# Zanue/EndoDAV

Measured on AMD Instinct MI355X. Metric: depth frames/sec (518x518, T=8 clip), higher is better.
Workload: dtype f32

## Files before the change

endodav_amd/_lib.py:

```python
from __future__ import annotations

import ctypes as C
import os
from typing import Optional

_HERE = os.path.dirname(os.path.abspath(__file__))
LIB_PATH = os.environ.get("EDV_LIB_PATH") or os.path.join(_HERE, "lib", "libendodav_hip.so")
ABI_VERSION = 15

LORA_TYPES = {"none": 0, "lora": 1, "dvlora": 2, "ssb": 3, "dash": 4}
ACT_NONE, ACT_GELU, ACT_RELU, ACT_SIGMOID, ACT_SIGMOID_NEG = 0, 1, 2, 3, 4


class EdvConfig(C.Structure):

    _fields_ = [
        ("abi_version", C.c_int32),
        ("embed_dim", C.c_int32),
        ("depth", C.c_int32),
        ("num_heads", C.c_int32),
        ("taps", C.c_int32 * 4),
        ("features", C.c_int32),
        ("out_channels", C.c_int32 * 4),
        ("image_h", C.c_int32),
# ... 29 lines not shown
    "edv_forward": (C.c_int, [C.c_void_p, _fp, _i32, _i32, _i32, _i32, C.POINTER(C.c_void_p), C.c_void_p]),
    "edv_output_shape": (C.c_int, [C.c_void_p, _i32, C.POINTER(_i32), C.POINTER(_i32)]),
    "edv_stage_copy": (C.c_int, [C.c_void_p, C.c_char_p, _fp, C.POINTER(C.c_size_t), C.c_void_p]),
    "edv_set_capture": (C.c_int, [C.c_void_p, C.c_int]),
    "edv_profile_enable": (C.c_int, [C.c_void_p, C.c_uint32]),
    "edv_set_encoder_streams": (C.c_int, [C.c_void_p, _i32]),
    "edv_set_products": (C.c_int, [C.c_void_p, _i32, C.c_void_p]),
    "edv_get_products": (C.c_int, [C.c_void_p]),
    "edv_profile_set_mask": (C.c_int, [C.c_void_p, C.c_uint32]),
    "edv_profile_work": (C.c_int, [C.c_void_p, _i32, C.POINTER(_f64), C.POINTER(_f64)]),
    "edv_profile_read": (C.c_int, [C.c_void_p, _i32, C.POINTER(_i32), C.POINTER(_f64)]),
    "edv_device_bytes": (C.c_size_t, [C.c_void_p]),
    "edv_last_launch_count": (C.c_int, [C.c_void_p]),
    "edv_layernorm": (C.c_int, [_fp, _fp, _fp, _fp, _i64, _i32, _f32, _fp, _i32, _i32, C.c_void_p]),
    "edv_gemm_workspace": (C.c_size_t, []),
    "edv_gemm_x6_planes_bytes": (C.c_size_t, [_i32, _i32]),
    "edv_gemm_x6_split": (C.c_int, [_fp, C.c_void_p, _i32, _i32, C.c_void_p]),
    "edv_gemm_x6": (C.c_int, [_fp, C.c_void_p, _fp, _i64, _i32, _i32, _fp, _i32, _fp, _fp, _fp, C.c_size_t, C.c_void_p]),
    "edv_gemm": (C.c_int, [_fp, _fp, _fp, _i64, _i32, _i32, _fp, _i32, _fp, _fp, _fp, C.c_size_t, C.c_void_p]),
    "edv_pack_geglu": (C.c_int, [_fp, _fp, _fp, _fp, _i32, _i32, C.c_void_p]),
    "edv_gemm_geglu": (C.c_int, [_fp, _fp, _fp, _fp, _i64, _i32, _i32, C.c_void_p]),
    "edv_conv3x3": (C.c_int, [_fp, _fp, _fp, _fp, _i32, _i32, _i32, _i32, _i32, _i32, _i32, _i32, _fp, _fp, C.c_void_p]),
    "edv_conv3x3_ws": (C.c_int, [_fp, _fp, _fp, _fp, _i32, _i32, _i32, _i32, _i32, _i32, _i32, _i32, _fp, _fp, _fp, C.c_size_t, C.c_void_p]),
    "edv_pack_conv3x3": (C.c_int, [_fp, _fp, _i32, _i32, C.c_void_p]),
    "edv_conv_transpose": (C.c_int, [_fp, _fp, _fp, _fp, _fp, _fp, _i32, _i32, _i32, _i32, _i32, C.c_void_p]),
    "edv_attn_spatial_workspace": (C.c_size_t, [_i32, _i32, _i32]),
    "edv_attn_spatial": (C.c_int, [_fp, _fp, _i32, _i32, _i32, _fp, C.c_size_t, _fp, C.c_void_p]),
    "edv_set_train": (C.c_int, [C.c_void_p, _i32]),
    "edv_set_grad_scope": (C.c_int, [C.c_void_p, _i32, _i32, _i32, _i32]),
    "edv_set_bias_grads": (C.c_int, [C.c_void_p, _i32, _i32]),
    "edv_generation": (C.c_int, [C.c_void_p, C.POINTER(C.c_uint64)]),
    "edv_backward": (C.c_int, [C.c_void_p, C.c_uint64, _fp, C.POINTER(C.c_void_p), C.c_void_p]),
    "edv_grad_bind_flat": (C.c_int, [C.c_void_p, _i32, C.POINTER(C.c_char_p), C.POINTER(_i64), _fp, _i64, C.POINTER(_i64)]),
    "edv_grad": (C.c_int, [C.c_void_p, C.c_char_p, C.POINTER(C.c_void_p), C.POINTER(_i64)]),
    "edv_grad_copy": (C.c_int, [C.c_void_p, C.c_char_p, _fp, _i64, C.c_void_p]),
    "edv_attn_spatial_x6_workspace": (C.c_size_t, [_i32, _i32, _i32]),
    "edv_attn_spatial_x6": (C.c_int, [_fp, _fp, _i32, _i32, _i32, _fp, C.c_size_t, C.c_void_p]),
    "edv_attn_spatial_bwd_workspace": (C.c_size_t, [_i32, _i32, _i32]),
    "edv_attn_spatial_bwd": (C.c_int, [_fp, _fp, _fp, _fp, _fp, _fp, _i32, _i32, _i32, _fp, C.c_size_t, C.c_void_p]),
    "edv_layernorm_bwd": (C.c_int, [_fp, _fp, _fp, _fp, _i64, _i32, C.c_float, _i32, C.c_void_p]),
    "edv_ew_bwd": (C.c_int, [_fp, _fp, _fp, _fp, _i64, _i32, C.c_void_p]),
    "edv_geglu_bwd": (C.c_int, [_fp, _fp, _fp, _i64, _i32, C.c_void_p]),
    "edv_transpose_scale": (C.c_int, [_fp, _fp, _fp, _i32, _i32, C.c_void_p]),
    "edv_lora_grads_workspace": (C.c_size_t, [_i64, _i32, _i32, _i32]),
    "edv_lora_grads": (C.c_int, [_fp, _fp, _i64, _i32, _i32, _i32, _fp, _fp, _fp, _fp, C.c_float, _fp, _fp, C.c_size_t, _fp, _fp, _fp, _fp, C.c_void_p]),
    "edv_bilinear_bwd": (C.c_int, [_fp, _fp, _i32, _i32, _i32, _i32, _i32, _i32, _i32, C.c_void_p]),
# ... 128 lines not shown
```

endodav_amd/csrc/api.hip:

```cpp
#include "../../include/endodav_hip.h"
#include <algorithm>
#include <vector>

#include "ops.hpp"

using namespace edv;

extern "C" {

int edv_layernorm(const float *x_dev, const float *w_dev, const float *b_dev, float *y_dev, int64_t rows, int32_t dim, float eps,
                  const float *pe_dev, int32_t rows_per_frame, int32_t T, void *stream) {
    return layernorm(x_dev, identity_map(), w_dev, b_dev, y_dev, identity_map(), rows, dim, eps, pe_dev, rows_per_frame, T, (hipStream_t)stream);
}

size_t edv_gemm_workspace(void) { return gemm_workspace() * sizeof(float); }
int edv_gemm(const float *A_dev, const float *W_dev, float *C_dev, int64_t M, int32_t N, int32_t K, const float *bias_dev, int32_t act,
             const float *gamma_dev, const float *R_dev, float *workspace_dev, size_t workspace_bytes, void *stream) {
    GemmDesc g;
    g.A = A_dev; g.lda = K; g.W = W_dev; g.ldw = K; g.C = C_dev; g.ldc = N; g.M = M; g.N = N; g.K = K;
    g.bias = bias_dev; g.act = act; g.gamma = gamma_dev; g.R1 = R_dev; g.ldr1 = N;
    g.ws = workspace_dev; g.ws_floats = workspace_bytes / sizeof(float);
    EDV_CHECK(act >= ACT_NONE && act <= ACT_RELU, "act must be 0, 1 or 2");
    return gemm(g, (hipStream_t)stream);
}
// ... 33 lines not shown
                        int32_t Cout, int32_t stride, int32_t pre_relu, int32_t post_relu, const float *R1_dev, const float *R2_dev, float *ws,
                        size_t ws_bytes, void *stream) {
    EDV_CHECK(F > 0 && H > 0 && W > 0 && Cin > 0 && Cout > 0, "empty problem");
    EDV_CHECK(stride == 1 || stride == 2, "stride must be 1 or 2");
    GemmDesc g;
    const int OH = (H - 1) / stride + 1, OW = (W - 1) / stride + 1;
    g.A = x_dev; g.W = wpacked_dev; g.ldw = 9 * Cin; g.C = y_dev; g.ldc = Cout; g.M = (long long)F * OH * OW; g.N = Cout; g.K = 9 * Cin;
    g.bias = bias_dev; g.act = post_relu ? ACT_RELU : ACT_NONE; g.R1 = R1_dev; g.ldr1 = Cout; g.R2 = R2_dev; g.ldr2 = Cout;
    g.loader = LOAD_CONV3; g.cH = H; g.cW = W; g.cC = Cin; g.cOH = OH; g.cOW = OW; g.cS = stride; g.pre_relu = pre_relu ? 1 : 0;
    g.ws = ws; g.ws_floats = ws_bytes / sizeof(float);
    return gemm(g, (hipStream_t)stream);
}

int edv_conv3x3(const float *x_dev, const float *wpacked_dev, const float *bias_dev, float *y_dev, int32_t F, int32_t H, int32_t W, int32_t Cin,
                int32_t Cout, int32_t stride, int32_t pre_relu, int32_t post_relu, const float *R1_dev, const float *R2_dev, void *stream) {
    return conv3x3_impl(x_dev, wpacked_dev, bias_dev, y_dev, F, H, W, Cin, Cout, stride, pre_relu, post_relu, R1_dev, R2_dev, nullptr, 0, stream);
}

int edv_conv3x3_ws(const float *x_dev, const float *wpacked_dev, const float *bias_dev, float *y_dev, int32_t F, int32_t H, int32_t W, int32_t Cin,
                   int32_t Cout, int32_t stride, int32_t pre_relu, int32_t post_relu, const float *R1_dev, const float *R2_dev, float *workspace_dev,
                   size_t workspace_bytes, void *stream) {
    return conv3x3_impl(x_dev, wpacked_dev, bias_dev, y_dev, F, H, W, Cin, Cout, stride, pre_relu, post_relu, R1_dev, R2_dev, workspace_dev,
                        workspace_bytes, stream);
}

int edv_pack_conv3x3(const float *w_dev, float *wpacked_dev, int32_t Cout, int32_t Cin, void *stream) {
    return pack_conv3x3(w_dev, wpacked_dev, Cout, Cin, (hipStream_t)stream);
}

int edv_conv_transpose(const float *x_dev, const float *w_dev, const float *b_dev, float *wpack_dev, float *bpack_dev, float *y_dev, int32_t F, int32_t h,
              int32_t w, int32_t C, int32_t s, void *stream) {
    EDV_CHECK(F > 0 && h > 0 && w > 0 && C > 0 && s > 0, "empty problem");
    EDV_TRY(pack_convT(w_dev, wpack_dev, b_dev, bpack_dev, C, C, s, (hipStream_t)stream));
    GemmDesc g;
    g.A = x_dev; g.lda = C; g.W = wpack_dev; g.ldw = C; g.C = y_dev; g.ldc = C; g.M = (long long)F * h * w; g.N = s * s * C; g.K = C;
    g.bias = bpack_dev; g.store = STORE_SHUFFLE; g.ps_s = s; g.ps_C = C; g.ps_h = h; g.ps_w = w;
    return gemm(g, (hipStream_t)stream);
}

size_t edv_attn_spatial_workspace(int32_t F, int32_t N, int32_t heads) { return attn_spatial_workspace(F, N, heads) * sizeof(float); }
int edv_attn_spatial(const float *qkv_dev, float *out_dev, int32_t F, int32_t N, int32_t heads, float *workspace_dev, size_t workspace_bytes,
                     float *lse_dev, void *stream) {
    return attn_spatial(qkv_dev, out_dev, F, N, heads, workspace_dev, workspace_bytes / sizeof(float), (hipStream_t)stream, lse_dev);
}
size_t edv_attn_spatial_x6_workspace(int32_t F, int32_t N, int32_t heads) { return attn_spatial_workspace(F, N, heads, true) * sizeof(float); }
int edv_attn_spatial_x6(const float *qkv_dev, float *out_dev, int32_t F, int32_t N, int32_t heads, float *workspace_dev, size_t workspace_bytes, void *stream) {
// ... 336 lines not shown
```

endodav_amd/csrc/conv_dma.hip:

```cpp
#include <cstdlib>
#include <type_traits>

#include "gemm_common.hpp"

namespace edv {
namespace {

constexpr int CBK = 32;
__device__ __attribute__((aligned(256))) float g_zero_page[64];

template <int WGM, int EP, bool SPLIT, bool BUF>
__global__ __launch_bounds__(256, 4) void conv3_dma_kernel(const GemmDesc g, const GemmSplit sp) {
    constexpr int WGN = 4 / WGM;
    constexpr int BM = 32 * WGM, BN = 32 * WGN;
    constexpr int IA = BM / 32, IB = BN / 32;
    constexpr int STAGE = (BM + BN) * CBK;
    __shared__ __attribute__((aligned(16))) float smem[2 * STAGE];
    const int tid = threadIdx.x, lane = tid & 63, wave = tid >> 6, l31 = lane & 31, lh = lane >> 5;
    const int wave_s = __builtin_amdgcn_readfirstlane(wave);
    const bool prelu = g.pre_relu != 0;
    const int wm = wave / WGN, wn = wave % WGN;
    const int tiles_n = (g.N + BN - 1) / BN;
    const int bid = xcd_remap(blockIdx.x, gridDim.x);
    const unsigned a_bytes = BUF ? (unsigned)((g.M > 0 ? ((g.M - 1) / (g.cOH * g.cOW) + 1) : 0) * (long long)g.cH * g.cW * g.cC * 4) : 0u;
// ... 98 lines not shown
                    __builtin_amdgcn_global_load_lds((const __attribute__((address_space(1))) void *)src,
                                                     (__attribute__((address_space(3))) void *)(sA + ((BM / 4) * wave + 8 * i) * CBK), 16, 0, 0);
                }
            }
#pragma unroll
            for (int i = 0; i < IB; ++i) {
                if constexpr (BUF)
                    __builtin_amdgcn_raw_ptr_buffer_load_lds(rW, (__attribute__((address_space(3))) void *)(sB + ((BN / 4) * wave_s + 8 * i) * CBK), 16, (unsigned)vb[i], (int)(k * 4), 0,
                                                             0);
                else
                    __builtin_amdgcn_global_load_lds((const __attribute__((address_space(1))) void *)(pb[i] + k),
                                                     (__attribute__((address_space(3))) void *)(sB + ((BN / 4) * wave + 8 * i) * CBK), 16, 0, 0);
            }
        };
        const float *fpa[4], *fpb[4];
#pragma unroll
        for (int q = 0; q < 4; ++q) {
            fpa[q] = smem + ra * CBK + (((2 * q + lh) ^ swa) << 2);
            fpb[q] = smem + BM * CBK + rb * CBK + (((2 * q + lh) ^ swb) << 2);
        }

        EpiCols<1> cols;
        if (EP != 0) cols = gemm_epilogue_prefetch<1>(g, n0, wn * 32, l31);
        f32x16 acc[1][1];
        auto epilogue = [&]() {
            if constexpr (BUF && EP >= 1 && EP <= 3)
                gemm_epilogue_buf<EP - 1>(g, acc[0][0], cols, m0 + (wave_s / WGN) * 32, n0 + (wave_s % WGN) * 32, l31, lh);
            else
                gemm_epilogue_ep<1, 1, STORE_ROWS, EP>(g, acc, cols, m0, n0, wm * 32, wn * 32, l31, lh);
        };
#pragma unroll
        for (int r = 0; r < 16; ++r) acc[0][0][r] = 0.f;

        issue(kt0, 0);
        asm volatile("s_waitcnt vmcnt(0)" ::: "memory");
        __builtin_amdgcn_s_barrier();
        auto ktile = [&](int kt, auto st_tag) {
            constexpr int ST = decltype(st_tag)::value;
            if (kt + 1 < kt1) issue(kt + 1, ST ^ 1);
            f32x4 fa[4], fb[4];
#pragma unroll
            for (int q = 0; q < 4; ++q) {
                fa[q] = *reinterpret_cast<const f32x4 *>(fpa[q] + ST * STAGE);
                fb[q] = *reinterpret_cast<const f32x4 *>(fpb[q] + ST * STAGE);
            }
            __builtin_amdgcn_sched_barrier(0);
            if (prelu) {
#pragma unroll
                for (int q = 0; q < 4; ++q)
// ... 84 lines not shown
            launch_variant<WGM, EP, true>(d, sp, buf, (unsigned)grid, st);
            EDV_LAUNCH_OK();
            return 0;
        }
        grid = tiles;
    }
    launch_variant<WGM, EP, false>(d, sp, buf, (unsigned)grid, st);
    EDV_LAUNCH_OK();
    return 0;
}

template <int WGM>
int launch_conv(const GemmDesc &d, hipStream_t st) {
    constexpr int BM = 32 * WGM, BN = 32 * (4 / WGM);
    const long long tiles = ((d.M + BM - 1) / BM) * (long long)((d.N + BN - 1) / BN);
    EDV_CHECK(tiles > 0 && tiles < (1ll << 31), "bad grid");
    switch (epilogue_kind(d)) {
        case 1: return launch_conv_ep<WGM, 1>(d, tiles, st);
        case 3: return launch_conv_ep<WGM, 3>(d, tiles, st);
        default: return launch_conv_ep<WGM, 0>(d, tiles, st);
    }
}

}

const SplitPolicy &conv_dma_split_policy() {
    static const SplitPolicy p{.min_kt = 18, .min_tiles = 16, .max_rounds = 0, .widen = false, .counters = SPLIT_MAX_COUNTERS, .slot_floats = SPLIT_SLOT,
                               .whole_rounds = false, .deep_kt = 48, .idle_factor = 8};
    return p;
}

bool conv_dma_supported(const GemmDesc &d) {
    return d.loader == LOAD_CONV3 && d.store == STORE_ROWS && d.cC % CBK == 0 && d.K == 9 * d.cC && d.ldw % 4 == 0 && d.M > 0 && d.N > 0;
}

int conv_dma(const GemmDesc &d, hipStream_t st) {
    EDV_CHECK(d.A && d.W && d.C, "null operand");
    EDV_CHECK(conv_dma_supported(d), "LDS-DMA convolution needs Cin % 32 == 0");
    EDV_CHECK(((uintptr_t)d.A % 16 == 0) && ((uintptr_t)d.W % 16 == 0), "A/W must be 16-byte aligned");
    return d.N <= 32 ? launch_conv<4>(d, st) : launch_conv<2>(d, st);
}

}
```

endodav_amd/csrc/engine_forward.hip:

```cpp
#include "engine.hpp"

namespace {

struct OnStream {
    Run &r;
    const hipStream_t st;
    float *const skws;
    const int F;
    OnStream(Run &run, hipStream_t s, float *ws) : r(run), st(run.st), skws(run.skws), F(run.F) { r.st = s; r.skws = ws; }
    ~OnStream() { r.st = st; r.skws = skws; r.F = F; }
};

struct Forward : Run {
    using Run::Run;
    std::string rb_suffix;
    int enc_F = 0, enc_f0 = 0;
    bool stagger_record = false;
    float *tap[4], *tapcls[4] = {nullptr, nullptr, nullptr, nullptr}, *pj[4], *lv[4], *rn[4], *path[5], *readout = nullptr, *fbias = nullptr;

    int pos_table(const float **out) {
        const float *pos;
        EDV_TRY(param("pretrained.pos_embed", &pos, 3));
        const int Npos = cfg.pos_tokens - 1;
        const int npatch = ntok - 1;
// ... 554 lines not shown
            EDV_TRY(skip_branch(3, rn[2], h3, w3, u[3]));
        }
        EDV_HIP(hipEventRecord(c->ev_x[2], side));
        EDV_TRY(level(0));
        EDV_TRY(level(1));
        EDV_HIP(hipEventRecord(c->ev_x[1], user));
        EDV_HIP(hipStreamWaitEvent(side, c->ev_x[1], 0));
        {
            OnStream side_(*this, side, ws_side);
            EDV_TRY(skip_branch(2, rn[1], h2, w2, u[2]));
            EDV_HIP(hipEventRecord(c->ev_x[3], side));
            EDV_TRY(skip_branch(1, rn[0], h1, w1, u[1]));
        }
        EDV_HIP(hipEventRecord(c->ev_x[4], side));
        EDV_HIP(hipStreamWaitEvent(user, c->ev_join[0], 0));
        return fuse(u);
    }

    int depth_head(const std::string &tg, const std::string &c1, const std::string &c2, const std::string &c3, const float *x, int h, int w, int oh,
                   int ow, size_t cap_in, size_t cap_out, int act, float *out) {
        float *o1, *up, *o2;
        EDV_TRY(wsbuf(tg + "o1", cap_in * Fh, &o1));
        EDV_TRY(wsbuf(tg + "up", cap_out * Fh, &up));
        EDV_TRY(wsbuf(tg + "o2", cap_out * 32, &o2));
        const float *wt, *b;
        EDV_TRY(packedw(c1 + ".weight", &wt));
        EDV_TRY(param(c1 + ".bias", &b));
        EDV_TRY(conv3(x, h, w, Fe, wt, b, Fh, 1, o1, false));
        {
            HbmScope b_(c, KC_BILINEAR, st, 4.0 * (double)F * Fh * ((double)h * w + (double)oh * ow));
            EDV_TRY(bilinear(o1, up, F, h, w, Fh, oh, ow, ACT_NONE, st));
        }
        EDV_TRY(packedw(c2 + ".weight", &wt));
        EDV_TRY(param(c2 + ".bias", &b));
        EDV_TRY(conv3(up, oh, ow, Fh, wt, b, 32, 1, o2, false, ACT_RELU));
        EDV_TRY(param(c3 + ".weight", &wt));
        EDV_TRY(param(c3 + ".bias", &b));
        c->launches += 2;
        HbmScope b_(c, KC_DOT, st, 4.0 * (double)F * oh * ow * 33);
        return dot_channels(o2, wt, b, out, (long long)F * oh * ow, 32, act, st);
    }
    int vda_head(float *const disp[4]) {
        const int ih = cfg.image_h, iw = cfg.image_w;
        const std::string oc = "head.scratch.output_conv";
        EDV_TRY(depth_head("hd.", oc + "1", oc + "2.0", oc + "2.2", path[1], h0, w0, ih, iw, (size_t)F * h0 * w0, (size_t)F * ih * iw, ACT_RELU, disp[0]));
        int sh = ih, sw = iw;
        for (int k = 1; k < 4; ++k) {
            const int nh = sh / 2, nw = sw / 2;
            HbmScope b_(c, KC_BILINEAR, st, 4.0 * (double)F * ((double)sh * sw + (double)nh * nw));
            EDV_TRY(bilinear(disp[k - 1], disp[k], F, sh, sw, 1, nh, nw, ACT_NONE, st));
            sh = nh; sw = nw;
        }
        c->launches += 3;
        if (cfg.out_sigmoid) {
            if (c->train) {
// ... 67 lines not shown
```

endodav_amd/csrc/gemm_common.hpp:

```cpp
#pragma once
#include "ops.hpp"

namespace edv {

using f32x16 = __attribute__((ext_vector_type(16))) float;
using f32x4 = __attribute__((ext_vector_type(4))) float;

__device__ __forceinline__ float apply_act(float v, int act) {
    if (act == ACT_GELU) return gelu_erf(v);
    if (act == ACT_RELU) return fmaxf(v, 0.0f);
    return v;
}

#ifndef EDV_SPLIT_ACQUIRE
#define EDV_SPLIT_ACQUIRE 1
#endif
__device__ __forceinline__ void split_merge_acquire() {
#if EDV_SPLIT_ACQUIRE
    __builtin_amdgcn_fence(__ATOMIC_ACQUIRE, "agent");
    asm volatile("s_waitcnt vmcnt(0)" ::: "memory");
#endif
}
constexpr int SPLIT_SLOT = 64 * 64;
constexpr int SPLIT_MAX_COUNTERS = 4096;
// ... 204 lines not shown
        for (int r = 0; r < 16; ++r)
            res[r >> 1][r & 1] += __uint_as_float(__builtin_amdgcn_raw_buffer_load_b32(rs, (int)vo, (int)(so + (unsigned)(((r & 3) + 8 * (r >> 2)) * g.ldr2 * 4)), 0));
    }
    const unsigned lane_out = col0 + l31 >= g.N ? 0xfffff000u : 0u;
    const auto rc = __builtin_amdgcn_make_buffer_rsrc(g.C, 0, (int)(unsigned)(g.M * g.ldc * 4), 0x00020000);
    const unsigned vo = (unsigned)((4 * lh * g.ldc + l31) * 4) | lane_out;
    const unsigned so = (unsigned)((row0 * g.ldc + col0) * 4);
    const f32x2 bias = {cols.bias[0], cols.bias[0]}, gam = {cols.gam[0], cols.gam[0]};
#pragma unroll
    for (int i = 0; i < 8; ++i) {
        f32x2 v = f32x2{acc[2 * i], acc[2 * i + 1]} + bias;
        if (ACT == ACT_GELU) v = f32x2{gelu_erf(v[0]), gelu_erf(v[1])};
        if (ACT == ACT_RELU) v = f32x2{fmaxf(v[0], 0.0f), fmaxf(v[1], 0.0f)};
        v = v * gam + res[i];
#pragma unroll
        for (int e = 0; e < 2; ++e) {
            const int r = 2 * i + e;
            const float ve = e ? v[1] : v[0];
            __builtin_amdgcn_raw_buffer_store_b32(__float_as_uint(ve), rc, (int)vo, (int)(so + (unsigned)(((r & 3) + 8 * (r >> 2)) * g.ldc * 4)), EDV_EPI_STORE_AUX);
        }
    }
}

template <int FM, int FN>
__device__ __forceinline__ void gemm_epilogue_mapped(const GemmDesc &g, f32x16 (&acc)[FM][FN], const EpiCols<FN> &cols, long long m0, int n0, int wrow,
                                                     int wcol, int l31, int lh) {
    const int P = g.c_map.period;
#pragma unroll
    for (int j = 0; j < FN; ++j) {
        const int n = n0 + wcol + j * 32 + l31;
        if (n >= g.N) continue;
        const float bias = cols.bias[j], gam = cols.gam[j];
#pragma unroll
        for (int i = 0; i < FM; ++i) {
            const long long mb = m0 + wrow + i * 32 + 4 * lh;
            const int left = (int)(g.M - mb < 32 ? g.M - mb : 32);
            const long long f0 = mb / P;
            const int in0 = (int)(mb - f0 * P);
#pragma unroll
            for (int r = 0; r < 16; ++r) {
                const int dr = (r & 3) + 8 * (r >> 2);
                if (dr >= left) continue;
                const int t = in0 + dr;
                const int wrap = t >= P ? 1 : 0;
                const long long f = f0 + wrap;
                const int pin = t - wrap * P;
// ... 21 lines not shown
```

endodav_amd/csrc/ops.hpp:

```cpp
#pragma once
#include "common.hpp"
#include "streamk_plan.hpp"

namespace edv {

enum { ACT_NONE = 0, ACT_GELU = 1, ACT_RELU = 2, ACT_SIGMOID = 3, ACT_SIGMOID_NEG = 4 };
enum { LOAD_DENSE = 0, LOAD_CONV3 = 1 };
enum { STORE_ROWS = 0, STORE_SHUFFLE = 1 };

struct GemmDesc {
    const float *A = nullptr;
    int lda = 0;
    RowMap a_map{0, 0, 0};
    const float *W = nullptr;
    int ldw = 0;
    float *C = nullptr;
    int ldc = 0;
    RowMap c_map{0, 0, 0};
    long long M = 0;
    int N = 0, K = 0;
    const float *bias = nullptr;
    int act = ACT_NONE;
    const float *gamma = nullptr;
    const float *R1 = nullptr;
    int ldr1 = 0;
    RowMap r1_map{0, 0, 0};
    const float *R2 = nullptr;
    int ldr2 = 0;
    const float *P1 = nullptr;
    int ldp1 = 0;
    RowMap p1_map{0, 0, 0};
    int loader = LOAD_DENSE;
    int cH = 0, cW = 0, cC = 0, cOH = 0, cOW = 0, cS = 1, pre_relu = 0;
    int store = STORE_ROWS;
    int geglu = 0;
    int ps_s = 0, ps_C = 0, ps_h = 0, ps_w = 0;
    float *ws = nullptr;
    size_t ws_floats = 0;
    const void *Wx6 = nullptr;
};
int gemm(const GemmDesc &d, hipStream_t st);
size_t gemm_x6_planes_bytes(int N, int K);
int gemm_x6_split(const float *W, void *planes, int N, int K, hipStream_t st);
bool gemm_x6_supported(const GemmDesc &d);
int gemm_x6(const GemmDesc &d, hipStream_t st);
size_t gemm_workspace();
size_t gemm_counter_bytes();
bool gemm_dma_supported(const GemmDesc &d);
bool gemm_geglu_supported(const GemmDesc &d);
int pack_geglu(const float *w, const float *b, float *wi, float *bi, int N, int K, hipStream_t st);
int gemm_dma(const GemmDesc &d, hipStream_t st);
bool conv_dma_supported(const GemmDesc &d);
int conv_dma(const GemmDesc &d, hipStream_t st);
const SplitPolicy &gemm_dma_split_policy();
const SplitPolicy &gemm_x6_split_policy();
const SplitPolicy &conv_dma_split_policy();
const char *gemm_kernel_name(const GemmDesc &d);

size_t attn_spatial_workspace(int F, int N, int heads, bool x6 = false);
int attn_spatial(const float *qkv, float *out, int F, int N, int heads, float *ws, size_t ws_floats, hipStream_t st, float *lse = nullptr, bool x6 = false);
size_t attn_spatial_bwd_workspace(int F, int N, int heads);
int attn_spatial_bwd(const float *qkv, const float *out, const float *dout, const float *lse, float *delta, float *dqkv, int F, int N, int heads, float *ws,
                     size_t ws_floats, hipStream_t st);
int attn_temporal(const float *qkv, float *out, int B, int T, int P, int C, int heads, hipStream_t st);
int geglu(const float *x, float *y, long long M, int inner, hipStream_t st);
int rope_qk(float *qkv, const float *table, int B, int T, int P, int C, bool transpose, hipStream_t st);

int layernorm(const float *x, RowMap in_map, const float *w, const float *b, float *y, RowMap out_map, long long rows, int dim,
              float eps, const float *pe, int rows_per_frame, int T, hipStream_t st, int act = ACT_NONE, bool accumulate = false);
size_t groupnorm_workspace(int F, int P, int C);
int groupnorm(const float *x, const float *w, const float *b, float *y, float *stats, int F, int P, int C, int groups, float eps, hipStream_t st,
              float *part = nullptr, size_t part_floats = 0);

int patchify(const float *x, float *cols, int F, int H, int W, int ih, int iw, hipStream_t st, int ld = 588)  ;
int bilinear(const float *x, float *y, int F, int H, int W, int C, int OH, int OW, int act, hipStream_t st, const float *add = nullptr);
int dot_channels(const float *x, const float *w, const float *b, float *y, long long M, int C, int act, hipStream_t st);
// ... 114 lines not shown
```

include/endodav_hip.h:

```cpp
#ifndef ENDODAV_HIP_H
#define ENDODAV_HIP_H

#include <stddef.h>
#include <stdint.h>

#ifdef __cplusplus
extern "C" {
#endif

#define EDV_ABI_VERSION 15

enum edv_lora_type { EDV_LORA_NONE = 0, EDV_LORA_LORA = 1, EDV_LORA_DVLORA = 2, EDV_LORA_SSB = 3, EDV_LORA_DASH = 4 };

typedef struct edv_config {
    int32_t abi_version;
    int32_t embed_dim;
    int32_t depth;
    int32_t num_heads;
    int32_t taps[4];
    int32_t features;
    int32_t out_channels[4];
    int32_t image_h, image_w;
    int32_t num_frames;
    int32_t pos_tokens;
// ... 41 lines not shown
int edv_last_launch_count(const edv_ctx *ctx);


int edv_layernorm(const float *x_dev, const float *w_dev, const float *b_dev, float *y_dev, int64_t rows, int32_t dim,
                  float eps, const float *pe_dev, int32_t rows_per_frame, int32_t T, void *stream);

int edv_gemm(const float *A_dev, const float *W_dev, float *C_dev, int64_t M, int32_t N, int32_t K, const float *bias_dev,
             int32_t act, const float *gamma_dev, const float *R_dev, float *workspace_dev, size_t workspace_bytes, void *stream);
size_t edv_gemm_workspace(void);
size_t edv_gemm_x6_planes_bytes(int32_t N, int32_t K);
int edv_gemm_x6_split(const float *W_dev, void *planes_dev, int32_t N, int32_t K, void *stream);
int edv_gemm_x6(const float *A_dev, const void *planes_dev, float *C_dev, int64_t M, int32_t N, int32_t K, const float *bias_dev, int32_t act,
                const float *gamma_dev, const float *R_dev, float *workspace_dev, size_t workspace_bytes, void *stream);

int edv_pack_geglu(const float *w_dev, const float *b_dev, float *wi_dev, float *bi_dev, int32_t N, int32_t K, void *stream);
int edv_gemm_geglu(const float *A_dev, const float *Wi_dev, const float *bi_dev, float *C_dev, int64_t M, int32_t N, int32_t K, void *stream);

int edv_conv3x3(const float *x_dev, const float *wpacked_dev, const float *bias_dev, float *y_dev, int32_t F, int32_t H, int32_t W,
                int32_t Cin, int32_t Cout, int32_t stride, int32_t pre_relu, int32_t post_relu, const float *R1_dev,
                const float *R2_dev, void *stream);
int edv_conv3x3_ws(const float *x_dev, const float *wpacked_dev, const float *bias_dev, float *y_dev, int32_t F, int32_t H, int32_t W,
                   int32_t Cin, int32_t Cout, int32_t stride, int32_t pre_relu, int32_t post_relu, const float *R1_dev,
                   const float *R2_dev, float *workspace_dev, size_t workspace_bytes, void *stream);
int edv_pack_conv3x3(const float *w_dev, float *wpacked_dev, int32_t Cout, int32_t Cin, void *stream);

size_t edv_attn_spatial_workspace(int32_t F, int32_t N, int32_t heads);
int edv_attn_spatial(const float *qkv_dev, float *out_dev, int32_t F, int32_t N, int32_t heads, float *workspace_dev,
                     size_t workspace_bytes, float *lse_dev, void *stream);
size_t edv_attn_spatial_x6_workspace(int32_t F, int32_t N, int32_t heads);
int edv_attn_spatial_x6(const float *qkv_dev, float *out_dev, int32_t F, int32_t N, int32_t heads, float *workspace_dev, size_t workspace_bytes,
                        void *stream);
size_t edv_attn_spatial_bwd_workspace(int32_t F, int32_t N, int32_t heads);
int edv_attn_spatial_bwd(const float *qkv_dev, const float *out_dev, const float *dout_dev, const float *lse_dev, float *delta_dev,
                         float *dqkv_dev, int32_t F, int32_t N, int32_t heads, float *workspace_dev, size_t workspace_bytes, void *stream);

int edv_attn_temporal(const float *qkv_dev, float *out_dev, int32_t B, int32_t T, int32_t P, int32_t C, int32_t heads, void *stream);

int edv_rope_qk(float *qkv_dev, const float *table_dev, int32_t B, int32_t T, int32_t P, int32_t C, int32_t transpose, void *stream);

size_t edv_groupnorm_workspace(int32_t F, int32_t P, int32_t C);
int edv_groupnorm(const float *x_dev, const float *w_dev, const float *b_dev, float *y_dev, float *stats_dev ,
                  int32_t F, int32_t P, int32_t C, int32_t groups, float eps, float *workspace_dev, size_t workspace_bytes, void *stream);

int edv_geglu(const float *x_dev, float *y_dev, int64_t M, int32_t inner, void *stream);

int edv_debug_fill_lds(float value, void *stream);
// ... 164 lines not shown
```

Measured before the change: 1070.

## Add halo-tiled 3x3 conv kernel and fuse final 1x1 conv into conv epilogue

Adds a halo-tiled stride-1 3x3 convolution kernel that loads an input patch with halo into LDS once and reuses it across all nine taps, used for large full-resolution convs with 32/64 input channels. It also fuses the depth head's final 1x1 conv (a dot over the 32 output channels plus bias and activation) into the 3x3 conv epilogue via cross-lane reductions. This avoids writing and re-reading the 32-channel intermediate at full resolution and saves a launch. It adds new code paths with more restrictive support conditions and a runtime switch.

```diff
diff --git a/endodav_amd/_lib.py b/endodav_amd/_lib.py
--- a/endodav_amd/_lib.py
+++ b/endodav_amd/_lib.py
@@ -75,6 +75,8 @@
     "edv_gemm_geglu": (C.c_int, [_fp, _fp, _fp, _fp, _i64, _i32, _i32, C.c_void_p]),
     "edv_conv3x3": (C.c_int, [_fp, _fp, _fp, _fp, _i32, _i32, _i32, _i32, _i32, _i32, _i32, _i32, _fp, _fp, C.c_void_p]),
     "edv_conv3x3_ws": (C.c_int, [_fp, _fp, _fp, _fp, _i32, _i32, _i32, _i32, _i32, _i32, _i32, _i32, _fp, _fp, _fp, C.c_size_t, C.c_void_p]),
+    "edv_set_conv_impl": (C.c_int, [_i32]),
+    "edv_conv3x3_dot": (C.c_int, [_fp, _fp, _fp, _fp, _i32, _i32, _i32, _i32, _i32, _i32, _i32, _i32, _fp, _fp, _i32, C.c_void_p]),
     "edv_pack_conv3x3": (C.c_int, [_fp, _fp, _i32, _i32, C.c_void_p]),
     "edv_conv_transpose": (C.c_int, [_fp, _fp, _fp, _fp, _fp, _fp, _i32, _i32, _i32, _i32, _i32, C.c_void_p]),
     "edv_attn_spatial_workspace": (C.c_size_t, [_i32, _i32, _i32]),
diff --git a/endodav_amd/csrc/api.hip b/endodav_amd/csrc/api.hip
--- a/endodav_amd/csrc/api.hip
+++ b/endodav_amd/csrc/api.hip
@@ -79,6 +79,26 @@
                    size_t workspace_bytes, void *stream) {
     return conv3x3_impl(x_dev, wpacked_dev, bias_dev, y_dev, F, H, W, Cin, Cout, stride, pre_relu, post_relu, R1_dev, R2_dev, workspace_dev,
                         workspace_bytes, stream);
+}
+
+int edv_set_conv_impl(int32_t mode) {
+    EDV_CHECK(mode >= 0 && mode <= 2, "edv_set_conv_impl: mode 0 (automatic), 1 (never fused) or 2 (fused wherever supported)");
+    set_conv_impl(mode);
+    return 0;
+}
+
+int edv_conv3x3_dot(const float *x_dev, const float *wpacked_dev, const float *bias_dev, float *y_dev, int32_t F, int32_t H, int32_t W, int32_t Cin,
+                    int32_t Cout, int32_t stride, int32_t pre_relu, int32_t post_relu, const float *w2_dev, const float *b2_dev, int32_t act2, void *stream) {
+    EDV_CHECK(F > 0 && H > 0 && W > 0 && Cin > 0 && Cout > 0, "empty problem");
+    EDV_CHECK(stride == 1 || stride == 2, "stride must be 1 or 2");
+    EDV_CHECK(conv_dot_enabled(), "edv_conv3x3_dot: the fused epilogue is switched off (edv_set_conv_impl(1) or EDV_CONV_DOT=0)");
+    GemmDesc g;
+    const int OH = (H - 1) / stride + 1, OW = (W - 1) / stride + 1;
+    g.A = x_dev; g.W = wpacked_dev; g.ldw = 9 * Cin; g.ldc = Cout; g.M = (long long)F * OH * OW; g.N = Cout; g.K = 9 * Cin;
+    g.bias = bias_dev; g.act = post_relu ? ACT_RELU : ACT_NONE;
+    g.loader = LOAD_CONV3; g.cH = H; g.cW = W; g.cC = Cin; g.cOH = OH; g.cOW = OW; g.cS = stride; g.pre_relu = pre_relu ? 1 : 0;
+    g.w2 = w2_dev; g.b2 = b2_dev; g.act2 = act2; g.dot_out = y_dev;
+    return conv_dot(g, (hipStream_t)stream);
 }
 
 int edv_pack_conv3x3(const float *w_dev, float *wpacked_dev, int32_t Cout, int32_t Cin, void *stream) {
diff --git a/endodav_amd/csrc/conv_dma.hip b/endodav_amd/csrc/conv_dma.hip
--- a/endodav_amd/csrc/conv_dma.hip
+++ b/endodav_amd/csrc/conv_dma.hip
@@ -1,3 +1,4 @@
+#include <atomic>
 #include <cstdlib>
 #include <type_traits>
 
@@ -144,9 +145,17 @@
 
         EpiCols<1> cols;
         if (EP != 0) cols = gemm_epilogue_prefetch<1>(g, n0, wn * 32, l31);
+        float w2v = 0.f, b2v = 0.f;
+        if constexpr (EP >= 8) {
+            w2v = g.w2[n0 + l31 < g.N ? n0 + l31 : g.N - 1];
+            if (g.b2) b2v = g.b2[0];
+        }
         f32x16 acc[1][1];
         auto epilogue = [&]() {
-            if constexpr (BUF && EP >= 1 && EP <= 3)
+            if constexpr (EP >= 8) {
+                static_assert(EP < 8 || (WGM == 4 && BUF && !SPLIT), "the fused 1x1 needs every column of a row in one wave, and 32-bit offsets");
+                gemm_epilogue_dot<EP - 8>(g, acc[0][0], cols, w2v, b2v, m0 + wave_s * 32, n0, l31, lh);
+            } else if constexpr (BUF && EP >= 1 && EP <= 3)
                 gemm_epilogue_buf<EP - 1>(g, acc[0][0], cols, m0 + (wave_s / WGN) * 32, n0 + (wave_s % WGN) * 32, l31, lh);
             else
                 gemm_epilogue_ep<1, 1, STORE_ROWS, EP>(g, acc, cols, m0, n0, wm * 32, wn * 32, l31, lh);
@@ -277,6 +286,31 @@
     }
 }
 
+std::atomic<int> g_conv_impl{0};
+
+bool dot_fits_buffer(const GemmDesc &d) {
+    const long long frames = (d.M - 1) / ((long long)d.cOH * d.cOW) + 1;
+    return frames * d.cH * d.cW * d.cC * 4 < (1ll << 31) - (1 << 20) && (long long)d.N * d.ldw * 4 < (1ll << 32) - (1 << 20) && (d.M + 128) * 4 < (1ll << 32) - (1 << 20);
+}
+
+template <int EP>
+int launch_conv_dot(const GemmDesc &d, hipStream_t st) {
+    const long long tiles = (d.M + 127) / 128;
+    EDV_CHECK(tiles > 0 && tiles < (1ll << 31), "bad grid");
+    GemmSplit sp{};
+    long long grid;
+    plan_plain(tiles, conv_dma_split_policy(), &sp, &grid);
+    EDV_LAUNCH((conv3_dma_kernel<4, EP, false, true>), dim3((unsigned)grid), dim3(256), 0, st, d, sp);
+    EDV_LAUNCH_OK();
+    return 0;
+}
+
+}
+
+void set_conv_impl(int mode) { g_conv_impl.store(mode < 0 || mode > 2 ? 0 : mode, std::memory_order_relaxed); }
+int conv_impl() { return g_conv_impl.load(std::memory_order_relaxed); }
+bool conv_dot_enabled() {
+    return conv_impl() != 1 && env_int("EDV_CONV_DOT", 1) != 0;
 }
 
 const SplitPolicy &conv_dma_split_policy() {
@@ -289,10 +323,24 @@
     return d.loader == LOAD_CONV3 && d.store == STORE_ROWS && d.cC % CBK == 0 && d.K == 9 * d.cC && d.ldw % 4 == 0 && d.M > 0 && d.N > 0;
 }
 
+bool conv_dot_supported(const GemmDesc &d) {
+    return conv_dma_supported(d) && d.N <= 32 && (d.act == ACT_NONE || d.act == ACT_RELU) && d.act2 != ACT_GELU && d.act2 >= ACT_NONE && d.act2 <= ACT_SIGMOID_NEG &&
+           !d.gamma && !d.R1 && !d.R2 && !d.P1 && d.c_map.period == 0 && dot_fits_buffer(d);
+}
+
+int conv_dot(const GemmDesc &d, hipStream_t st) {
+    EDV_CHECK(d.A && d.W && d.w2 && d.dot_out, "null operand");
+    EDV_CHECK(conv_dot_supported(d), "fused 1x1 epilogue: Cin % 32 == 0, Cout <= 32, post-activation none / ReLU, no residual, operands below 2 GB");
+    EDV_CHECK(((uintptr_t)d.A % 16 == 0) && ((uintptr_t)d.W % 16 == 0), "A/W must be 16-byte aligned");
+    if (conv_halo_wanted(d)) return conv_halo(d, st);
+    return d.act == ACT_RELU ? launch_conv_dot<8 + ACT_RELU>(d, st) : launch_conv_dot<8 + ACT_NONE>(d, st);
+}
+
 int conv_dma(const GemmDesc &d, hipStream_t st) {
     EDV_CHECK(d.A && d.W && d.C, "null operand");
     EDV_CHECK(conv_dma_supported(d), "LDS-DMA convolution needs Cin % 32 == 0");
     EDV_CHECK(((uintptr_t)d.A % 16 == 0) && ((uintptr_t)d.W % 16 == 0), "A/W must be 16-byte aligned");
+    if (conv_halo_wanted(d)) return conv_halo(d, st);
     return d.N <= 32 ? launch_conv<4>(d, st) : launch_conv<2>(d, st);
 }
 
diff --git a/endodav_amd/csrc/conv_halo.hip b/endodav_amd/csrc/conv_halo.hip
--- /dev/null
+++ b/endodav_amd/csrc/conv_halo.hip
@@ -0,0 +1,211 @@
+#include <cstdlib>
+#include <type_traits>
+
+#include "gemm_common.hpp"
+
+namespace edv {
+namespace {
+
+constexpr int HBK = 32;
+constexpr int TH = 8, TW = 16;
+constexpr int ROW_BYTES = 3 * 64 * 16;
+constexpr int PIX_BYTES = 9 * 16;
+constexpr int PLANE_BYTES = (TH + 2) * ROW_BYTES;
+constexpr int WSTAGE = 32 * HBK;
+constexpr unsigned LANE_OUT = 0x80000000u;
+constexpr unsigned ROW_OUT = 0x7ff00000u;
+
+template <int NCB, int ACT, bool DOT>
+__global__ __launch_bounds__(256, NCB == 1 ? 4 : 2) void conv3_halo_kernel(const GemmDesc g) {
+    __shared__ __attribute__((aligned(16))) float smem[2 * WSTAGE + NCB * PLANE_BYTES / 4];
+    constexpr int CIN = NCB * 32, NKT = 9 * NCB;
+    const int tid = threadIdx.x, lane = tid & 63, l31 = lane & 31, lh = lane >> 5;
+    const int wave_s = __builtin_amdgcn_readfirstlane(tid >> 6);
+    const bool prelu = g.pre_relu != 0;
+    const int H = g.cH, W = g.cW;
+    const int bid = xcd_remap(blockIdx.x, gridDim.x);
+    const int tiles_x = (W + TW - 1) / TW, tiles_y = (H + TH - 1) / TH;
+    const int f = bid / (tiles_x * tiles_y), tr = bid - f * (tiles_x * tiles_y);
+    const int ty = tr / tiles_x, tx = tr - ty * tiles_x;
+    const int oy0 = ty * TH, ox0 = tx * TW;
+    const int frames = (int)(g.M / ((long long)H * W));
+    const unsigned a_bytes = (unsigned)((long long)frames * H * W * CIN * 4);
+    const auto rA = __builtin_amdgcn_make_buffer_rsrc(const_cast<float *>(g.A), 0, a_bytes, 0x00020000);
+    const auto rW = __builtin_amdgcn_make_buffer_rsrc(const_cast<float *>(g.W), 0, 0xffffffff, 0x00020000);
+    float *const sW = smem;
+    char *const patch = reinterpret_cast<char *>(smem + 2 * WSTAGE);
+
+    unsigned pat[3];
+#pragma unroll
+    for (int k = 0; k < 3; ++k) {
+        const unsigned ci = (unsigned)(k * 64 + lane);
+        const unsigned hx = ci / 9u, c = ci - 9u * hx;
+        const int ix = ox0 - 1 + (int)hx;
+        pat[k] = (hx < (unsigned)(TW + 2) && c < 8u && ix >= 0 && ix < W) ? (unsigned)((ix * CIN + (int)c * 4) * 4) : LANE_OUT;
+    }
+#pragma unroll
+    for (int t = 0; t < ((TH + 2) * NCB + 3) / 4; ++t) {
+        const int u = wave_s + 4 * t;
+        if (u < (TH + 2) * NCB) {
+            const int cb = NCB == 1 ? 0 : u / (TH + 2), hy = u - cb * (TH + 2);
+            const int iy = oy0 - 1 + hy;
+            const unsigned so = (iy >= 0 && iy < H) ? (unsigned)((((f * H + iy) * W) * CIN + cb * 32) * 4) : ROW_OUT;
+            char *dst = patch + cb * PLANE_BYTES + hy * ROW_BYTES;
+#pragma unroll
+            for (int k = 0; k < 3; ++k)
+                __builtin_amdgcn_raw_ptr_buffer_load_lds(rA, (__attribute__((address_space(3))) void *)(dst + k * 1024), 16, (unsigned)pat[k], (int)so, 0, 0);
+        }
+    }
+    const int srow = lane >> 3, spos = lane & 7;
+    unsigned vb;
+    {
+        const int r = 8 * wave_s + srow;
+        const int c = spos ^ ((r >> 1) & 7);
+        const int n = r < g.N ? r : g.N - 1;
+        vb = (unsigned)((n * g.ldw + c * 4) * 4);
+    }
+    auto issue_w = [&](int kt, int stg) {
+        __builtin_amdgcn_raw_ptr_buffer_load_lds(rW, (__attribute__((address_space(3))) void *)(sW + stg * WSTAGE + 8 * wave_s * HBK), 16, (unsigned)vb, (int)(kt * HBK * 4),
+                                                 0, 0);
+    };
+    const int swb = (l31 >> 1) & 7;
+    const float *fpb[4];
+#pragma unroll
+    for (int q = 0; q < 4; ++q) fpb[q] = sW + l31 * HBK + (((2 * q + lh) ^ swb) << 2);
+    const char *const a0 = patch + (2 * wave_s) * ROW_BYTES + (l31 >> 4) * ROW_BYTES + (l31 & 15) * PIX_BYTES + lh * 16;
+
+    EpiCols<1> cols = gemm_epilogue_prefetch<1>(g, 0, 0, l31);
+    float w2v = 0.f, b2v = 0.f;
+    if constexpr (DOT) {
+        w2v = g.w2[l31 < g.N ? l31 : g.N - 1];
+        if (g.b2) b2v = g.b2[0];
+    }
+    f32x16 acc;
+#pragma unroll
+    for (int r = 0; r < 16; ++r) acc[r] = 0.f;
+
+    issue_w(0, 0);
+    asm volatile("s_waitcnt vmcnt(0)" ::: "memory");
+    __builtin_amdgcn_s_barrier();
+#pragma unroll
+    for (int kt = 0; kt < NKT; ++kt) {
+        const int stg = kt & 1, tap = kt / NCB, cb = kt - tap * NCB, dy = tap / 3, dx = tap - 3 * dy;
+        if (kt + 1 < NKT) issue_w(kt + 1, stg ^ 1);
+        f32x4 fa[4], fb[4];
+#pragma unroll
+        for (int q = 0; q < 4; ++q) {
+            fa[q] = *reinterpret_cast<const f32x4 *>(a0 + cb * PLANE_BYTES + dy * ROW_BYTES + dx * PIX_BYTES + q * 32);
+            fb[q] = *reinterpret_cast<const f32x4 *>(fpb[q] + stg * WSTAGE);
+        }
+        __builtin_amdgcn_sched_barrier(0);
+        if (prelu) {
+#pragma unroll
+            for (int q = 0; q < 4; ++q)
+#pragma unroll
+                for (int e = 0; e < 4; ++e) fa[q][e] = __builtin_amdgcn_fmed3f(fa[q][e], 0.f, __builtin_inff());
+        }
+#pragma unroll
+        for (int q = 0; q < 4; ++q) {
+#pragma unroll
+            for (int e = 0; e < 4; ++e) acc = __builtin_amdgcn_mfma_f32_32x32x2f32(fa[q][e], fb[q][e], acc, 0, 0, 0);
+        }
+        __builtin_amdgcn_sched_barrier(0);
+        asm volatile("s_waitcnt vmcnt(0)" ::: "memory");
+        asm volatile("s_waitcnt lgkmcnt(0)" ::: "memory");
+        __builtin_amdgcn_s_barrier();
+    }
+
+    const int oyw = oy0 + 2 * wave_s;
+    const unsigned mbase = (unsigned)((f * H + oyw) * W + ox0);
+    if constexpr (DOT) {
+        const float v = gemm_dot_reduce<ACT>(g, acc, cols, w2v, b2v, l31 < g.N, l31);
+        const int i = l31 & 15, r = 2 * i + (l31 >> 4);
+        const int py = r >> 3, px = (r & 3) + 8 * ((r >> 2) & 1) + 4 * lh;
+        const bool ok = i < 8 && oyw + py < H && ox0 + px < W;
+        const auto ro = __builtin_amdgcn_make_buffer_rsrc(g.dot_out, 0, (int)(unsigned)(g.M * 4), 0x00020000);
+        __builtin_amdgcn_raw_buffer_store_b32(__float_as_uint(v), ro, (int)(ok ? (unsigned)((py * W + px) * 4) : LANE_OUT), (int)(mbase * 4u), EDV_EPI_STORE_AUX);
+    } else {
+        using f32x2 = __attribute__((ext_vector_type(2))) float;
+        const int ld = g.ldc;
+        const unsigned lane_off = l31 >= g.N ? LANE_OUT : (unsigned)((4 * lh * ld + l31) * 4);
+        const int lim = W - ox0 - 4 * lh;
+        unsigned vo[8];
+#pragma unroll
+        for (int j = 0; j < 8; ++j) vo[j] = ((j & 3) + 8 * (j >> 2)) < lim ? lane_off : LANE_OUT;
+        unsigned so[16];
+#pragma unroll
+        for (int r = 0; r < 16; ++r)
+            so[r] = oyw + (r >> 3) < H ? (mbase + (unsigned)((r >> 3) * W + (r & 3) + 8 * ((r >> 2) & 1))) * (unsigned)(ld * 4) : ROW_OUT;
+        f32x2 res[8];
+#pragma unroll
+        for (int i = 0; i < 8; ++i) res[i] = f32x2{0.f, 0.f};
+        const int bytes = (int)(unsigned)(g.M * ld * 4);
+        if (g.R1) {
+            const auto rs = __builtin_amdgcn_make_buffer_rsrc(const_cast<float *>(g.R1), 0, bytes, 0x00020000);
+#pragma unroll
+            for (int r = 0; r < 16; ++r) res[r >> 1][r & 1] = __uint_as_float(__builtin_amdgcn_raw_buffer_load_b32(rs, (int)vo[(r & 3) + 4 * ((r >> 2) & 1)], (int)so[r], 0));
+        }
+        if (g.R2) {
+            const auto rs = __builtin_amdgcn_make_buffer_rsrc(const_cast<float *>(g.R2), 0, bytes, 0x00020000);
+#pragma unroll
+            for (int r = 0; r < 16; ++r) res[r >> 1][r & 1] += __uint_as_float(__builtin_amdgcn_raw_buffer_load_b32(rs, (int)vo[(r & 3) + 4 * ((r >> 2) & 1)], (int)so[r], 0));
+        }
+        const auto rc = __builtin_amdgcn_make_buffer_rsrc(g.C, 0, bytes, 0x00020000);
+        const f32x2 bias = {cols.bias[0], cols.bias[0]}, gam = {cols.gam[0], cols.gam[0]};
+#pragma unroll
+        for (int i = 0; i < 8; ++i) {
+            f32x2 v = f32x2{acc[2 * i], acc[2 * i + 1]} + bias;
+            if (ACT == ACT_RELU) v = f32x2{fmaxf(v[0], 0.0f), fmaxf(v[1], 0.0f)};
+            v = v * gam + res[i];
+#pragma unroll
+            for (int e = 0; e < 2; ++e) {
+                const int r = 2 * i + e;
+                const float ve = e ? v[1] : v[0];
+                __builtin_amdgcn_raw_buffer_store_b32(__float_as_uint(ve), rc, (int)vo[(r & 3) + 4 * ((r >> 2) & 1)], (int)so[r], EDV_EPI_STORE_AUX);
+            }
+        }
+    }
+}
+
+template <int NCB, int ACT>
+int launch_halo(const GemmDesc &d, unsigned grid, hipStream_t st) {
+    if (d.w2) EDV_LAUNCH((conv3_halo_kernel<NCB, ACT, true>), dim3(grid), dim3(256), 0, st, d);
+    else EDV_LAUNCH((conv3_halo_kernel<NCB, ACT, false>), dim3(grid), dim3(256), 0, st, d);
+    EDV_LAUNCH_OK();
+    return 0;
+}
+
+long long halo_tiles(const GemmDesc &d) { return (d.M / ((long long)d.cH * d.cW)) * ((d.cH + TH - 1) / TH) * (long long)((d.cW + TW - 1) / TW); }
+
+}
+
+bool conv_halo_supported(const GemmDesc &d) {
+    if (!conv_dma_supported(d) || d.cS != 1 || d.N > 32 || (d.cC != 32 && d.cC != 64)) return false;
+    if (d.M % ((long long)d.cH * d.cW) != 0 || halo_tiles(d) >= (1ll << 31)) return false;
+    const long long lim = (1ll << 31) - (1 << 20);
+    if (d.M * d.cC * 4 >= lim || (long long)d.N * d.ldw * 4 >= lim) return false;
+    if (d.w2) return d.M * 4 < lim;
+    const int ep = epilogue_kind(d);
+    if (ep != 1 + ACT_NONE && ep != 1 + ACT_RELU) return false;
+    if ((d.R1 && d.ldr1 != d.ldc) || (d.R2 && d.ldr2 != d.ldc)) return false;
+    return d.M * d.ldc * 4 < lim;
+}
+
+bool conv_halo_pays(const GemmDesc &d) { return (d.cC == 32 || d.cC == 64) && d.N <= 32 && halo_tiles(d) >= 4096; }
+
+bool conv_halo_wanted(const GemmDesc &d) {
+    if (conv_impl() == 1 || !conv_halo_supported(d) || env_int("EDV_CONV_HALO", 1) == 0) return false;
+    return conv_impl() == 2 || conv_halo_pays(d);
+}
+
+int conv_halo(const GemmDesc &d, hipStream_t st) {
+    EDV_CHECK(d.A && d.W && (d.w2 ? (const void *)d.dot_out : (const void *)d.C), "null operand");
+    EDV_CHECK(conv_halo_supported(d), "halo convolution: stride 1, Cin 32 or 64, Cout <= 32, operands below 2 GB");
+    EDV_CHECK(((uintptr_t)d.A % 16 == 0) && ((uintptr_t)d.W % 16 == 0), "A/W must be 16-byte aligned");
+    const unsigned grid = (unsigned)halo_tiles(d);
+    const bool relu = d.act == ACT_RELU;
+    if (d.cC == 32) return relu ? launch_halo<1, ACT_RELU>(d, grid, st) : launch_halo<1, ACT_NONE>(d, grid, st);
+    return relu ? launch_halo<2, ACT_RELU>(d, grid, st) : launch_halo<2, ACT_NONE>(d, grid, st);
+}
+
+}
diff --git a/endodav_amd/csrc/engine_forward.hip b/endodav_amd/csrc/engine_forward.hip
--- a/endodav_amd/csrc/engine_forward.hip
+++ b/endodav_amd/csrc/engine_forward.hip
@@ -600,7 +600,6 @@
         float *o1, *up, *o2;
         EDV_TRY(wsbuf(tg + "o1", cap_in * Fh, &o1));
         EDV_TRY(wsbuf(tg + "up", cap_out * Fh, &up));
-        EDV_TRY(wsbuf(tg + "o2", cap_out * 32, &o2));
         const float *wt, *b;
         EDV_TRY(packedw(c1 + ".weight", &wt));
         EDV_TRY(param(c1 + ".bias", &b));
@@ -609,6 +608,23 @@
             HbmScope b_(c, KC_BILINEAR, st, 4.0 * (double)F * Fh * ((double)h * w + (double)oh * ow));
             EDV_TRY(bilinear(o1, up, F, h, w, Fh, oh, ow, ACT_NONE, st));
         }
+        GemmDesc gd;
+        gd.A = up; gd.ldw = 9 * Fh; gd.ldc = 32; gd.M = (long long)F * oh * ow; gd.N = 32; gd.K = 9 * Fh; gd.act = ACT_RELU; gd.act2 = act; gd.dot_out = out;
+        gd.loader = LOAD_CONV3; gd.cH = oh; gd.cW = ow; gd.cC = Fh; gd.cOH = oh; gd.cOW = ow; gd.cS = 1;
+        if (!c->train && conv_dot_enabled() && conv_dot_supported(gd)) {
+            EDV_TRY(packedw(c2 + ".weight", &gd.W));
+            EDV_TRY(param(c2 + ".bias", &gd.bias));
+            EDV_TRY(param(c3 + ".weight", &gd.w2));
+            EDV_TRY(param(c3 + ".bias", &gd.b2));
+            c->launches += 2;
+            if (c->prof_mask & (1u << KC_CONV3)) {
+                c->prof_flops[KC_CONV3] += 2.0 * (double)gd.M * gd.N * gd.K;
+                c->prof_bytes[KC_CONV3] += 4.0 * ((double)gd.M * Fh + (double)gd.N * gd.K + (double)gd.M);
+            }
+            Bracket b_(c, KC_CONV3, st);
+            return conv_dot(gd, st);
+        }
+        EDV_TRY(wsbuf(tg + "o2", cap_out * 32, &o2));
         EDV_TRY(packedw(c2 + ".weight", &wt));
         EDV_TRY(param(c2 + ".bias", &b));
         EDV_TRY(conv3(up, oh, ow, Fh, wt, b, 32, 1, o2, false, ACT_RELU));
diff --git a/endodav_amd/csrc/gemm_common.hpp b/endodav_amd/csrc/gemm_common.hpp
--- a/endodav_amd/csrc/gemm_common.hpp
+++ b/endodav_amd/csrc/gemm_common.hpp
@@ -250,6 +250,48 @@
     }
 }
 
+template <int ACT>
+__device__ __forceinline__ float gemm_dot_reduce(const GemmDesc &g, const f32x16 &acc, const EpiCols<1> &cols, float w2v, float b2v, bool col_in, int l31) {
+    float t[16];
+#pragma unroll
+    for (int r = 0; r < 16; ++r) {
+        float v = acc[r] + cols.bias[0];
+        if (ACT == ACT_RELU) v = fmaxf(v, 0.0f);
+        t[r] = col_in ? w2v * v : 0.f;
+    }
+    float s[8];
+#pragma unroll
+    for (int i = 0; i < 8; ++i) {
+        const auto sw = __builtin_amdgcn_permlane16_swap(__float_as_uint(t[2 * i]), __float_as_uint(t[2 * i + 1]), false, false);
+        float v = __uint_as_float(sw[0]) + __uint_as_float(sw[1]);
+        v += __uint_as_float(__builtin_amdgcn_update_dpp(0, __float_as_uint(v), 0xB1, 0xf, 0xf, true));
+        v += __uint_as_float(__builtin_amdgcn_update_dpp(0, __float_as_uint(v), 0x4E, 0xf, 0xf, true));
+        v += __uint_as_float(__builtin_amdgcn_update_dpp(0, __float_as_uint(v), 0x141, 0xf, 0xf, true));
+        v += __uint_as_float(__builtin_amdgcn_update_dpp(0, __float_as_uint(v), 0x140, 0xf, 0xf, true));
+        s[i] = v;
+    }
+    const int i = l31 & 15;
+    float v = s[0];
+#pragma unroll
+    for (int k = 1; k < 8; ++k) v = i == k ? s[k] : v;
+    v += b2v;
+    if (g.act2 == ACT_RELU) v = fmaxf(v, 0.f);
+    else if (g.act2 == ACT_SIGMOID) v = 1.f / (1.f + expf(-v));
+    else if (g.act2 == ACT_SIGMOID_NEG) v = 1.f / (1.f + expf(v));
+    return v;
+}
+
+template <int ACT>
+__device__ __forceinline__ void gemm_epilogue_dot(const GemmDesc &g, f32x16 &acc, const EpiCols<1> &cols, float w2v, float b2v, long long row0, int col0, int l31,
+                                                  int lh) {
+    const float v = gemm_dot_reduce<ACT>(g, acc, cols, w2v, b2v, col0 + l31 < g.N, l31);
+    const int i = l31 & 15, r = 2 * i + (l31 >> 4);
+    const unsigned row = (unsigned)((r & 3) + 8 * (r >> 2) + 4 * lh);
+    const auto ro = __builtin_amdgcn_make_buffer_rsrc(g.dot_out, 0, (int)(unsigned)(g.M * 4), 0x00020000);
+    const unsigned vo = i < 8 ? row * 4u : 0xfffff000u;
+    __builtin_amdgcn_raw_buffer_store_b32(__float_as_uint(v), ro, (int)vo, (int)(unsigned)(row0 * 4), EDV_EPI_STORE_AUX);
+}
+
 template <int FM, int FN>
 __device__ __forceinline__ void gemm_epilogue_mapped(const GemmDesc &g, f32x16 (&acc)[FM][FN], const EpiCols<FN> &cols, long long m0, int n0, int wrow,
                                                      int wcol, int l31, int lh) {
diff --git a/endodav_amd/csrc/ops.hpp b/endodav_amd/csrc/ops.hpp
--- a/endodav_amd/csrc/ops.hpp
+++ b/endodav_amd/csrc/ops.hpp
@@ -38,6 +38,9 @@
     float *ws = nullptr;
     size_t ws_floats = 0;
     const void *Wx6 = nullptr;
+    const float *w2 = nullptr, *b2 = nullptr;
+    float *dot_out = nullptr;
+    int act2 = ACT_NONE;
 };
 int gemm(const GemmDesc &d, hipStream_t st);
 size_t gemm_x6_planes_bytes(int N, int K);
@@ -52,6 +55,14 @@
 int gemm_dma(const GemmDesc &d, hipStream_t st);
 bool conv_dma_supported(const GemmDesc &d);
 int conv_dma(const GemmDesc &d, hipStream_t st);
+bool conv_dot_supported(const GemmDesc &d);
+int conv_dot(const GemmDesc &d, hipStream_t st);
+bool conv_halo_supported(const GemmDesc &d);
+bool conv_halo_wanted(const GemmDesc &d);
+int conv_halo(const GemmDesc &d, hipStream_t st);
+void set_conv_impl(int mode);
+int conv_impl();
+bool conv_dot_enabled();
 const SplitPolicy &gemm_dma_split_policy();
 const SplitPolicy &gemm_x6_split_policy();
 const SplitPolicy &conv_dma_split_policy();
diff --git a/include/endodav_hip.h b/include/endodav_hip.h
--- a/include/endodav_hip.h
+++ b/include/endodav_hip.h
@@ -87,6 +87,10 @@
 int edv_conv3x3_ws(const float *x_dev, const float *wpacked_dev, const float *bias_dev, float *y_dev, int32_t F, int32_t H, int32_t W,
                    int32_t Cin, int32_t Cout, int32_t stride, int32_t pre_relu, int32_t post_relu, const float *R1_dev,
                    const float *R2_dev, float *workspace_dev, size_t workspace_bytes, void *stream);
+int edv_set_conv_impl(int32_t mode);
+int edv_conv3x3_dot(const float *x_dev, const float *wpacked_dev, const float *bias_dev, float *y_dev, int32_t F, int32_t H, int32_t W,
+                    int32_t Cin, int32_t Cout, int32_t stride, int32_t pre_relu, int32_t post_relu, const float *w2_dev,
+                    const float *b2_dev, int32_t act2, void *stream);
 int edv_pack_conv3x3(const float *w_dev, float *wpacked_dev, int32_t Cout, int32_t Cin, void *stream);
 
 size_t edv_attn_spatial_workspace(int32_t F, int32_t N, int32_t heads);
diff --git a/scratch/kb_conv_halo.py b/scratch/kb_conv_halo.py
--- /dev/null
+++ b/scratch/kb_conv_halo.py
@@ -0,0 +1,79 @@
+import ctypes as C
+import math
+import os
+import sys
+
+import torch
+
+sys.path.insert(0, os.path.dirname(os.path.dirname(os.path.abspath(__file__))))
+from endodav_amd import _lib
+
+lib = _lib.load()
+cuda = torch.device("cuda:0")
+REPS, ROUNDS = 30, 4
+
+
+def st():
+    return C.c_void_p(torch.cuda.current_stream().cuda_stream)
+
+
+def rnd(*shape, seed=0, scale=1.0):
+    g = torch.Generator().manual_seed(seed)
+    return ((torch.rand(*shape, generator=g) * 2 - 1) * scale).to(cuda)
+
+
+def timed(fn):
+    for _ in range(5):
+        fn()
+    torch.cuda.synchronize()
+    a, b = torch.cuda.Event(enable_timing=True), torch.cuda.Event(enable_timing=True)
+    a.record()
+    for _ in range(REPS):
+        fn()
+    b.record()
+    torch.cuda.synchronize()
+    return a.elapsed_time(b) / REPS * 1e3
+
+
+def run(name, Fr, H, W, Cin, Cout, post, tail):
+    x = rnd(Fr, H, W, Cin, seed=1)
+    w = rnd(Cout, Cin, 3, 3, seed=2, scale=1 / math.sqrt(9 * Cin))
+    b = rnd(Cout, seed=3, scale=0.1)
+    w2, b2 = rnd(Cout, seed=6), rnd(1, seed=7)
+    wp = torch.empty(Cout * 9 * Cin, device=cuda)
+    _lib.check(lib.edv_pack_conv3x3(w.data_ptr(), wp.data_ptr(), Cout, Cin, st()))
+    y = torch.empty((Fr, H, W, Cout), device=cuda)
+    d = torch.empty((Fr, H, W), device=cuda)
+
+    def conv():
+        _lib.check(lib.edv_conv3x3(x.data_ptr(), wp.data_ptr(), b.data_ptr(), y.data_ptr(), Fr, H, W, Cin, Cout, 1, 0, post, None, None, st()))
+
+    def conv_then_dot():
+        conv()
+        _lib.check(lib.edv_dot_channels(y.data_ptr(), w2.data_ptr(), b2.data_ptr(), d.data_ptr(), Fr * H * W, Cout, 2, st()))
+
+    def fused():
+        _lib.check(lib.edv_conv3x3_dot(x.data_ptr(), wp.data_ptr(), b.data_ptr(), d.data_ptr(), Fr, H, W, Cin, Cout, 1, 0, post, w2.data_ptr(), b2.data_ptr(), 2, st()))
+
+    variants = [("dma", 1, "1", conv), ("halo", 2, "1", conv)]
+    if tail:
+        variants += [("dma+dot_channels", 1, "1", conv_then_dot), ("dma_fused", 2, "0", fused), ("halo_fused", 2, "1", fused)]
+    res = {v[0]: [] for v in variants}
+    for _ in range(ROUNDS):
+        for vname, mode, halo, fn in variants:
+            os.environ["EDV_CONV_HALO"] = halo
+            _lib.check(lib.edv_set_conv_impl(mode))
+            res[vname].append(round(timed(fn), 1))
+    _lib.check(lib.edv_set_conv_impl(0))
+    os.environ.pop("EDV_CONV_HALO", None)
+    for vname, ts in res.items():
+        print(f"{name:28s} {vname:18s} mean {sum(ts) / len(ts):7.1f} us  min {min(ts):7.1f} max {max(ts):7.1f}  {ts}", flush=True)
+    return res
+
+
+out = {}
+if len(sys.argv) > 1 and sys.argv[1] == "vitb":
+    out["vitb16 conv2.0 64->32 518^2"] = run("vitb16 conv2.0 64->32 518^2", 16, 518, 518, 64, 32, 1, True)
+    sys.exit(0)
+out["output_conv2.0 32->32 518^2"] = run("output_conv2.0 32->32 518^2", 8, 518, 518, 32, 32, 1, True)
+out["output_conv1 64->32 296^2"] = run("output_conv1 64->32 296^2", 8, 296, 296, 64, 32, 0, False)
```

Result: faster. 1087 (median of 6 runs) (+1.6%).
